# dbandstra/zang

Hardware: AMD Instinct MI355X
Metric: voice-samples/sec (higher is better)
Workload: dtype f32

## Files before the change

### zang_amd/csrc/dsp.hip.h

```cpp
#pragma once
#include "zmath.hip.h"
#include "lanes.hip.h"

template <int W>
struct PulseKT {
    typename LaneT<W>::U ifreq, brpt;
    typename LaneT<W>::F gdf2 , col, cc121, cc212;
};
using PulseK = PulseKT<1>;

__device__ __forceinline__ void pulse_setup_freq(PulseK &k, float srf, float freq) {
    const float gain = 0.7f;
    k.ifreq = zf32_to_u32(srf * freq);
    k.gdf2 = (gain / zutof23(k.ifreq)) * 2.0f;
    k.cc121 = k.gdf2 * (k.col - 1.0f) + gain;
    k.cc212 = k.gdf2 * k.col - gain;
}
__device__ __forceinline__ void pulse_setup_color(PulseK &k, float color) {
    k.brpt = zftou32(zclamp01(color));
    k.col = zutof23(k.brpt);
}
__device__ __forceinline__ void pulse_setup(PulseKT<1> &k, float srf, float freq, float color) {
    pulse_setup_color(k, color);
    pulse_setup_freq(k, srf, freq);
}
__device__ __forceinline__ void pulse_setup(PulseKT<2> &k, float srf, zf2 freq, zf2 color) {
    PulseK a, b;
    pulse_setup(a, srf, freq.x, color.x);
    pulse_setup(b, srf, freq.y, color.y);
    k.ifreq = zu2{a.ifreq, b.ifreq}; k.brpt = zu2{a.brpt, b.brpt};
    k.gdf2 = zf2{a.gdf2, b.gdf2}; k.col = zf2{a.col, b.col};
    k.cc121 = zf2{a.cc121, b.cc121}; k.cc212 = zf2{a.cc212, b.cc212};
}

__device__ __forceinline__ zf2 zutof23(zu2 x) { return zbits_f((x >> 9) | 0x3f800000u) - 1.0f; }

template <int W>
__device__ __forceinline__ typename LaneT<W>::F pulse_sample(const PulseKT<W> &k, typename LaneT<W>::U cnt,
                                                             typename LaneT<W>::F gain, typename LaneT<W>::F ngain) {
    using F = typename LaneT<W>::F;
    using M = typename LaneT<W>::M;
    const F p = zutof23(cnt);
    const M b0 = cnt < k.brpt;
    const M b1 = (cnt - k.ifreq) < k.brpt;
    const M b2 = cnt < k.ifreq;
    const F sg = zsel(b0, gain, ngain);
    const F ramp = k.gdf2 * zsel(b0, p, k.col - p) - sg;
    const F flat = zsel(b2, zsel(b0, k.cc121, k.cc212), sg);
    return zsel(b0 == b1, flat, ramp);
}

template <int W>
__device__ __forceinline__ typename LaneT<W>::F pulse_sample(const PulseKT<W> &k, typename LaneT<W>::U cnt) {
    using F = typename LaneT<W>::F;
    return pulse_sample<W>(k, cnt, zsplat<F>(0.7f), zsplat<F>(-0.7f));
}

#if !defined(__HIPCC_RTC__)
typedef unsigned long long PulseRoll;
__device__ __forceinline__ PulseRoll pulse_roll_init(const PulseK &k, uint32_t cnt) {
    return __builtin_amdgcn_ballot_w64((cnt - k.ifreq) < k.brpt);
}
__device__ __forceinline__ float pulse_sample_roll(const PulseK &k, uint32_t cnt, PulseRoll &prev, float gain = 0.7f, float ngain = -0.7f) {
#if defined(ZH_NO_PULSE_ROLL)
    (void)prev;
    return pulse_sample<1>(k, cnt, gain, ngain);
#endif
    const float p = zutof23(cnt);
    const bool b0 = cnt < k.brpt;
    const bool b2 = cnt < k.ifreq;
    const float sg = b0 ? gain : ngain;
    const float ramp = k.gdf2 * (b0 ? p : k.col - p) - sg;
    const float flat = b2 ? (b0 ? k.cc121 : k.cc212) : sg;
    const PulseRoll m0 = __builtin_amdgcn_ballot_w64(b0);
    const bool same = __builtin_amdgcn_inverse_ballot_w64(~(m0 ^ prev));
    prev = m0;
    return same ? flat : ramp;
}
#endif

template <class F> struct SvfOutT { F l, b, h; };
using SvfOut = SvfOutT<float>;
constexpr float kSvfDcOffset = 3.814697265625e-6f;
template <class F>
__device__ __forceinline__ SvfOutT<F> svf_core(F &l, F &b, F in, F cut, F res) {
    l += cut * b - kSvfDcOffset;
    b += cut * (in - b * res - l);
    l += cut * b;
    const F h = in - b * res - l;
    b += cut * h;
    return SvfOutT<F>{l, b, h};
}
template <class F> struct SvfMidT { F l, b1; };
using SvfMid = SvfMidT<float>;
template <class F>
__device__ __forceinline__ SvfMidT<F> svf_core_mid(F &l, F &b, F in, F cut, F res) {
    l += cut * b - kSvfDcOffset;
    b += cut * (in - b * res - l);
    l += cut * b;
    const F b1 = b;
    const F h = in - b * res - l;
    b += cut * h;
    return SvfMidT<F>{l, b1};
}
template <class F>
__device__ __forceinline__ SvfOutT<F> svf_finish(F l, F b1, F in, F cut, F res) {
    const F h = in - b1 * res - l;
    return SvfOutT<F>{l, b1 + cut * h, h};
}
template <class F>
__device__ __forceinline__ SvfOutT<F> svf_step(F &l, F &b, F input, F cut, F res) {
    return svf_core(l, b, input + kSvfDcOffset, cut, res);
}
template <class F>
__device__ __forceinline__ F svf_lowpass_into_zero(F l, F b) { return zsplat<F>(0.0f) + (l + b * 0.0f); }

__device__ __forceinline__ float pink_step(float (&b)[7], float white) {
    b[0] = 0.99886f * b[0] + white * 0.0555179f;
    b[1] = 0.99332f * b[1] + white * 0.0750759f;
    b[2] = 0.96900f * b[2] + white * 0.1538520f;
    b[3] = 0.86650f * b[3] + white * 0.3104856f;
    b[4] = 0.55000f * b[4] + white * 0.5329522f;
    b[5] = -0.7616f * b[5] - white * 0.0168980f;
    const float out = b[0] + b[1] + b[2] + b[3] + b[4] + b[5] + b[6] + white * 0.5362f;
    b[6] = white * 0.115926f;
    return out;
}
```

### zang_amd/csrc/nice.hip.h

```cpp
#pragma once
#include "common.hip.h"
#include "zmath.hip.h"
#include "dsp.hip.h"
#include "seq.hip.h"
#include "envelope.hip.h"
#include "voices.hip.h"

template <int W>
struct NiceLaneT {
    using F = typename LaneT<W>::F;
    using U = typename LaneT<W>::U;
    using M = typename LaneT<W>::M;
    U cnt;
    PulseKT<W> k;
    M bad;
    F g, ng;
    F l, b, cut, res;
    EnvLaneT<W, ZH_CURVE_CUBED> env;

    __device__ __forceinline__ void begin(float sample_rate, float srf, float sr8, F freq, F color, M note_on, M new_note) {
        bad = zor(freq < zsplat<F>(0.0f), freq > zsplat<F>(sr8));
        pulse_setup(k, srf, freq, color);
        const F zf = zsplat<F>(0.0f);
        const typename LaneT<W>::U zu = zsplatu<typename LaneT<W>::U>(0u);
        k.ifreq = zsel(bad, zu, k.ifreq); k.brpt = zsel(bad, zu, k.brpt);
        k.gdf2 = zsel(bad, zf, k.gdf2); k.cc121 = zsel(bad, zf, k.cc121); k.cc212 = zsel(bad, zf, k.cc212);
        g = zsel(bad, zf, zsplat<F>(0.7f)); ng = zsel(bad, zf, zsplat<F>(-0.7f));
        const F f8 = freq * 8.0f;
#pragma unroll
        for (int c = 0; c < W; c++) zput(cut, c, zclampf(zcutoff_from_frequency(zget(f8, c), sample_rate), 0.0f, 1.0f));
        res = zsplat<F>(1.0f - zclampf(0.7f, 0.0f, 1.0f));
        env.sample_rate = sample_rate;
        env.sustain_volume = zsplat<F>(0.8f);
        env.attack = CurvePT<W>{ZH_CURVE_CUBED, zsplat<F>(0.01f)};
        env.decay = CurvePT<W>{ZH_CURVE_CUBED, zsplat<F>(0.1f)};
        env.release = CurvePT<W>{ZH_CURVE_CUBED, zsplat<F>(0.5f)};
        env.note_on = note_on;
        env.begin(new_note);
    }

    __device__ __forceinline__ F osc(U c) const {
        const F pv = pulse_sample<W>(k, c, g, ng);
        return pv * 0.5f;
    }
    template <bool INTO_ZERO = false>
    __device__ __forceinline__ F tail_filter(F t0) {
        const SvfOutT<F> s = svf_step(l, b, t0, cut, res);
        if constexpr (INTO_ZERO) return s.l + s.b * 0.0f;
        else return svf_lowpass_into_zero(s.l, s.b);
    }
    __device__ __forceinline__ F tail_env() { return env.frame_masked(); }
    template <bool INTO_ZERO = false>
    __device__ __forceinline__ F tail(F t0) {
        const F t1 = tail_filter<INTO_ZERO>(t0);
        const F e0 = tail_env();
        return e0 * t1;
    }
    template <bool INTO_ZERO = false>
    __device__ __forceinline__ F frame() {
        const F t0 = osc(cnt);
        cnt = cnt + k.ifreq;
        return tail<INTO_ZERO>(t0);
    }
    __device__ __forceinline__ F env_quiet() const { return zbits_f(zbits_u(zsplat<F>(0.0f) + env.sustain_volume) & env.m_painted); }
    template <bool INTO_ZERO = false>
    __device__ __forceinline__ F frame_quiet(F e0) {
        const F t0 = osc(cnt);
        cnt = cnt + k.ifreq;
        return e0 * tail_filter<INTO_ZERO>(t0);
    }
    template <bool INTO_ZERO = false>
    __device__ __forceinline__ F frame_roll(PulseRoll &roll) { return tail<INTO_ZERO>(osc_next(roll)); }
    template <bool INTO_ZERO = false>
    __device__ __forceinline__ F frame_quiet_roll(F e0, PulseRoll &roll) { return e0 * tail_filter<INTO_ZERO>(osc_next(roll)); }
    __device__ __forceinline__ void roll_begin(PulseRoll &roll) const {
        static_assert(W == 1, "lane masks: one voice per lane");
        roll = pulse_roll_init(k, cnt);
    }
    __device__ __forceinline__ F osc_next(PulseRoll &roll) {
        const F pv = pulse_sample_roll(k, cnt, roll, g, ng);
        cnt = cnt + k.ifreq;
        return pv * 0.5f;
    }
};
using NiceLane = NiceLaneT<1>;

struct NiceArgs {
    float *color;
    uint32_t *cnt;
    float *fl, *fb;
    uint32_t *estate;
    float *et, *elast, *estart;
    uint32_t V;
    float sample_rate, srf, sr8;
    F32P freq;
    BoolP note_on, nic;
};

template <int W>
__device__ __forceinline__ void nice_load_state(NiceLaneT<W> &n, const NiceArgs &a, uint32_t v) {
    n.cnt = zload_u<W>(a.cnt, v); n.l = zload_f<W>(a.fl, v); n.b = zload_f<W>(a.fb, v);
    n.env.state = zload_u<W>(a.estate, v); n.env.t = zload_f<W>(a.et, v);
    n.env.last_value = zload_f<W>(a.elast, v); n.env.start = zload_f<W>(a.estart, v);
}
template <int W>
__device__ __forceinline__ void nice_load(NiceLaneT<W> &n, const NiceArgs &a, uint32_t v) {
    nice_load_state(n, a, v);
    n.begin(a.sample_rate, a.srf, a.sr8, zget_f32p<W>(a.freq, v), zload_f<W>(a.color, v), zget_boolp<W>(a.note_on, v), zget_boolp<W>(a.nic, v));
}
template <int W>
__device__ __forceinline__ void nice_store(NiceLaneT<W> &n, const NiceArgs &a, uint32_t v) {
    zstore_u<W>(a.cnt, v, n.cnt); zstore_f<W>(a.fl, v, n.l); zstore_f<W>(a.fb, v, n.b);
    zstore_u<W>(a.estate, v, n.env.state); zstore_f<W>(a.et, v, n.env.t);
    zstore_f<W>(a.elast, v, n.env.last_value); zstore_f<W>(a.estart, v, n.env.start);
}
```

### zang_amd/csrc/nice_mix.hip.h

```cpp
#pragma once
#include "nice.hip.h"
#ifndef ZH_K
#define ZH_K(name) name
#endif
constexpr int MIXF = 32;
constexpr int MIXS = 68;

template <int C, class G2>
__device__ __forceinline__ void nice_mix_gains(G2 &g2, const F32P &gain_l, const F32P &gain_r, bool live, uint32_t v, uint32_t wave, uint32_t rh) {
    typedef float f2 __attribute__((ext_vector_type(2)));
    if constexpr (C == 2) {
        __shared__ f2 gains[512];
        gains[threadIdx.x] = live ? f2{gain_l.get(v), gain_r.get(v)} : f2{0.0f, 0.0f};
        __syncthreads();
        const f2 *mine = &gains[wave * 64 + rh * 32];
#pragma unroll
        for (int j = 0; j < 32; j++) g2[j] = mine[j];
    }
}

template <int C, bool ROLL, int NW, class G2>
__device__ __forceinline__ void nice_mix_frames(NiceLane &n, PulseRoll &roll, const G2 &g2, float (*tile)[MIXS], float *__restrict__ pw_paint,
                                                size_t channel_stride, uint32_t rows, uint32_t wrow, uint32_t start, uint32_t end, uint32_t lane,
                                                uint32_t rf, uint32_t rh, float (*wsum)[NW ? NW : 4][C][MIXF] = nullptr, uint32_t wave = 0, uint32_t first = 0xFFFFFFFFu) {
    constexpr bool WG = NW != 0;
    uint32_t parity = 0;
    for (uint32_t f0 = first == 0xFFFFFFFFu ? start : first; f0 < end; f0 += MIXF) {
        const bool whole = f0 + MIXF <= end;
        if (!__any(n.env.mode == ENV_MODE_TOWARD)) {
            const float e0 = n.env_quiet();
            if (whole) {
#pragma unroll 4
                for (int k = 0; k < MIXF; k++) {
                    const float x = 0.0f + (ROLL ? n.template frame_quiet_roll<true>(e0, roll) : n.template frame_quiet<true>(e0));
                    tile[k][lane] = x;
                }
            } else {
                for (int k = 0; k < MIXF; k++) {
                    float x = 0.0f;
                    if (__builtin_amdgcn_readfirstlane((int)(f0 + k < end))) x = 0.0f + (ROLL ? n.template frame_quiet_roll<true>(e0, roll) : n.template frame_quiet<true>(e0));
                    tile[k][lane] = x;
                }
            }
        } else if (whole && n.env.quiet(MIXF)) {
            if (__all(n.env.mode == ENV_MODE_TOWARD)) {
#pragma unroll 4
                for (int k = 0; k < MIXF; k++) {
                    const float e0 = n.env.frame_masked_all_toward_quiet();
                    const float x = 0.0f + (ROLL ? n.template frame_quiet_roll<true>(e0, roll) : n.template frame_quiet<true>(e0));
                    tile[k][lane] = x;
                }
            } else {
#pragma unroll 4
                for (int k = 0; k < MIXF; k++) {
                    const float e0 = n.env.frame_masked_quiet();
                    const float x = 0.0f + (ROLL ? n.template frame_quiet_roll<true>(e0, roll) : n.template frame_quiet<true>(e0));
                    tile[k][lane] = x;
                }
            }
        } else if (whole) {
#pragma unroll 4
            for (int k = 0; k < MIXF; k++) {
                const float x = 0.0f + (ROLL ? n.template frame_roll<true>(roll) : n.template frame<true>());
                tile[k][lane] = x;
            }
        } else {
            for (int k = 0; k < MIXF; k++) {
                float x = 0.0f;
                if (__builtin_amdgcn_readfirstlane((int)(f0 + k < end))) x = 0.0f + (ROLL ? n.template frame_roll<true>(roll) : n.template frame<true>());
                tile[k][lane] = x;
            }
        }
        __builtin_amdgcn_fence(__ATOMIC_RELEASE, "wavefront");
        __builtin_amdgcn_wave_barrier();
        __builtin_amdgcn_fence(__ATOMIC_ACQUIRE, "wavefront");
        {
            const float4 *row4 = reinterpret_cast<const float4 *>(&tile[rf][rh * 32]);
            float row[32];
#pragma unroll
            for (int q = 0; q < 8; q++) { const float4 x = row4[q]; row[4 * q] = x.x; row[4 * q + 1] = x.y; row[4 * q + 2] = x.z; row[4 * q + 3] = x.w; }
            float sl, sr = 0.0f;
            if constexpr (C == 1) {
                sl = row[0];
#pragma unroll
                for (int j = 1; j < 32; j++) sl += row[j];
            } else {
                sl = row[0] * g2[0].x; sr = row[0] * g2[0].y;
#pragma unroll
                for (int j = 1; j < 32; j++) { sl += row[j] * g2[j].x; sr += row[j] * g2[j].y; }
            }
            const float hl = __shfl_down(sl, 32);
            const float hr = C == 2 ? __shfl_down(sr, 32) : 0.0f;
            if constexpr (!WG) {
                if (rh == 0 && f0 + rf < end) {
                    const uint32_t fr = (f0 - start) + rf;
                    float *pw = pw_paint + ((size_t)(fr / kMixGroupFrames) * rows + wrow) * kMixGroupFrames + (fr % kMixGroupFrames);
                    pw[0] = sl + hl;
                    if constexpr (C == 2) pw[channel_stride] = sr + hr;
                }
            } else {
                if (rh == 0) {
                    wsum[parity][wave][0][rf] = sl + hl;
                    if constexpr (C == 2) wsum[parity][wave][1][rf] = sr + hr;
                }
                __syncthreads();
                constexpr uint32_t FW = MIXF / (NW ? NW : 4);
                static_assert(kMixGroupFrames % FW == 0, "a wave's frames stay inside one frame group");
                const uint32_t q = lane % FW, c = lane / FW, fw = wave * FW + q;
                if (c < (uint32_t)C && f0 + fw < end) {
                    float t = wsum[parity][0][c][fw] + wsum[parity][1][c][fw];
#pragma unroll
                    for (int w = 2; w < (NW ? NW : 4); w++) t += wsum[parity][w][c][fw];
                    const uint32_t fr = (f0 - start) + fw;
                    pw_paint[c * channel_stride + ((size_t)(fr / kMixGroupFrames) * rows + wrow) * kMixGroupFrames + (fr % kMixGroupFrames)] = t;
                }
                parity ^= 1u;
            }
        }
        __builtin_amdgcn_fence(__ATOMIC_RELEASE, "wavefront");
        __builtin_amdgcn_wave_barrier();
    }
}

__device__ __forceinline__ void nice_silence(NiceLane &n) {
    n.k.ifreq = 0u; n.k.brpt = 0u; n.k.gdf2 = 0.0f; n.k.cc121 = 0.0f; n.k.cc212 = 0.0f; n.g = n.ng = 0.0f;
    n.l = n.b = 0.0f;
    n.env.mode = ENV_MODE_NONE; n.env.m_painted = 0u;
}

template <int C, bool ROLL, int NW = 0>
__global__ void __launch_bounds__(NW == 8 ? 512 : 256) ZH_K(k_nice_mix)(NiceArgs a, uint32_t start, uint32_t end, float *__restrict__ partials,
                                                                  F32P gain_l, F32P gain_r) {
    constexpr bool WG = NW != 0;
    constexpr int NWV = NW ? NW : 4;
    __shared__ float tile_all[NWV][MIXF][MIXS];
    __shared__ float wsum[WG ? 2 : 1][NWV][C][MIXF];
    const uint32_t v = blockIdx.x * (NWV * 64) + threadIdx.x;
    const uint32_t lane = threadIdx.x & 63, wave = threadIdx.x >> 6;
    float (*tile)[MIXS] = tile_all[wave];
    const uint32_t nframes = end - start;
    const uint32_t wave_global = WG ? blockIdx.x : blockIdx.x * NWV + wave;
    const uint32_t rows = WG ? gridDim.x : gridDim.x * NWV;
    const size_t channel_stride = (size_t)((nframes + kMixGroupFrames - 1) / kMixGroupFrames) * rows * kMixGroupFrames;
    const bool live = v < a.V;
    NiceLane n;
    nice_load(n, a, live ? v : a.V - 1);
    if (!live) nice_silence(n);
    const uint32_t rf = lane & (MIXF - 1), rh = lane >> 5;
    PulseRoll roll;
    n.roll_begin(roll);
    typedef float f2 __attribute__((ext_vector_type(2)));
    f2 g2[C == 2 ? 32 : 1];
    nice_mix_gains<C>(g2, gain_l, gain_r, live, v, wave, rh);
    nice_mix_frames<C, ROLL, NW>(n, roll, g2, tile, partials, channel_stride, rows, wave_global, start, end, lane, rf, rh, wsum, wave);
    if (live) nice_store(n, a, v);
}

constexpr int kNiceMixMaxBatch = 16;
struct NiceBatchArgs {
    NiceArgs a;
    F32P freq[kNiceMixMaxBatch];
    BoolP note_on[kNiceMixMaxBatch], nic[kNiceMixMaxBatch];
    uint32_t nb;
};
template <int C, bool ROLL, int NW = 0>
__global__ void __launch_bounds__(NW == 8 ? 512 : 256) ZH_K(k_nice_mix_batch)(const NiceBatchArgs b, uint32_t start, uint32_t end, float *__restrict__ partials,
                                                                        F32P gain_l, F32P gain_r) {
    constexpr bool WG = NW != 0;
    constexpr int NWV = NW ? NW : 4;
    __shared__ float tile_all[NWV][MIXF][MIXS];
    __shared__ float wsum[WG ? 2 : 1][NWV][C][MIXF];
    const NiceArgs &a = b.a;
    const uint32_t v = blockIdx.x * (NWV * 64) + threadIdx.x;
    const uint32_t lane = threadIdx.x & 63, wave = threadIdx.x >> 6;
    float (*tile)[MIXS] = tile_all[wave];
    const uint32_t nframes = end - start;
    const uint32_t wave_global = WG ? blockIdx.x : blockIdx.x * NWV + wave;
    const uint32_t rows = WG ? gridDim.x : gridDim.x * NWV;
    const size_t channel_stride = (size_t)((nframes + kMixGroupFrames - 1) / kMixGroupFrames) * rows * kMixGroupFrames;
    const bool live = v < a.V;
    const uint32_t vc = live ? v : a.V - 1;
    NiceLane n;
    nice_load_state(n, a, vc);
    const float color = a.color[vc];
    const uint32_t rf = lane & (MIXF - 1), rh = lane >> 5;
    typedef float f2 __attribute__((ext_vector_type(2)));
    f2 g2[C == 2 ? 32 : 1];
    nice_mix_gains<C>(g2, gain_l, gain_r, live, v, wave, rh);
    for (uint32_t k = 0; k < b.nb; k++) {
        n.begin(a.sample_rate, a.srf, a.sr8, b.freq[k].get(vc), color, b.note_on[k].get(vc), b.nic[k].get(vc));
        if (!live) nice_silence(n);
        PulseRoll roll;
        n.roll_begin(roll);
        nice_mix_frames<C, ROLL, NW>(n, roll, g2, tile, partials + (size_t)k * C * channel_stride, channel_stride, rows, wave_global, start, end, lane, rf, rh, wsum, wave);
    }
    if (live) nice_store(n, a, v);
}

void zh_nice_mix_fma_launch(int channels, bool roll, int nw, uint32_t blocks, hipStream_t st, const NiceArgs &a, uint32_t start, uint32_t end,
                            float *part, F32P gl, F32P gr);
void zh_nice_mix_batch_fma_launch(bool roll, int nw, uint32_t blocks, hipStream_t st, const NiceBatchArgs &bt, uint32_t start, uint32_t end,
                                  float *part, F32P gl, F32P gr);
```

### zang_amd/csrc/zmath.hip.h

```cpp
#pragma once
#include <hip/hip_runtime.h>
#if !defined(__HIPCC_RTC__)
#include <stdint.h>
#endif
#include "rtc_types.hip.h"

#define ZD __device__ __forceinline__

ZD uint32_t zf2u(float f) { return __float_as_uint(f); }
ZD float zu2f(uint32_t u) { return __uint_as_float(u); }

ZD uint32_t zf32_to_u32(float v) {
#if defined(__HIP_DEVICE_COMPILE__)
    uint32_t r;
    asm("v_cvt_u32_f32 %0, %1" : "=v"(r) : "v"(v));
    return r;
#else
    if (!(v == v)) return 0u;
    if (v <= 0.0f) return 0u;
    if (v >= 4294967296.0f) return 0xFFFFFFFFu;
    return (uint32_t)v;
#endif
}
ZD int32_t zf32_to_i32(float v) {
#if defined(__HIP_DEVICE_COMPILE__)
    int32_t r;
    asm("v_cvt_i32_f32 %0, %1" : "=v"(r) : "v"(v));
    return r;
#else
    if (!(v == v)) return 0;
    if (v <= -2147483648.0f) return INT32_MIN;
    if (v >= 2147483648.0f) return INT32_MAX;
    return (int32_t)v;
#endif
}

ZD float zminf(float a, float b) { return (a <= b || b != b) ? a : b; }
ZD float zmaxf(float a, float b) { return (a >= b || b != b) ? a : b; }
ZD float zclampf(float v, float lo, float hi) { return zmaxf(lo, zminf(v, hi)); }

__device__ static const int32_t ZM_IPIO2[66] = {
  0xA2F983, 0x6E4E44, 0x1529FC, 0x2757D1, 0xF534DD, 0xC0DB62,
  0x95993C, 0x439041, 0xFE5163, 0xABDEBB, 0xC561B7, 0x246E3A,
  0x424DD2, 0xE00649, 0x2EEA09, 0xD1921C, 0xFE1DEB, 0x1CB129,
  0xA73EE8, 0x8235F5, 0x2EBB44, 0x84E99C, 0x7026B4, 0x5F7E41,
  0x3991D6, 0x398353, 0x39F49C, 0x845F8B, 0xBDF928, 0x3B1FF8,
  0x97FFDE, 0x05980F, 0xEF2F11, 0x8B5A0A, 0x6D1F6D, 0x367ECF,
  0x27CB09, 0xB74F46, 0x3F669E, 0x5FEA2D, 0x7527BA, 0xC7EBE5,
  0xF17B3D, 0x0739F7, 0x8A5292, 0xEA6BFB, 0x5FB11F, 0x8D5D08,
  0x560330, 0x46FC7B, 0x6BABF0, 0xCFBC20, 0x9AF436, 0x1DA9E3,
  0x91615E, 0xE61B08, 0x659985, 0x5F14A0, 0x68408D, 0xFFD880,
  0x4D7327, 0x310606, 0x1556CA, 0x73A8C9, 0x60E27B, 0xC08C6B,
};
__device__ static const double ZM_PIO2[8] = {
  0x1.921fb40000000p+0,  0x1.4442d00000000p-24, 0x1.8469880000000p-48,
  0x1.8cc5160000000p-72, 0x1.01b8380000000p-96, 0x1.a252040000000p-120,
  0x1.3822280000000p-145, 0x1.9f31d00000000p-169,
};

struct ZRemLarge { int n; double y; };
__device__ __noinline__ __attribute__((pure)) static ZRemLarge zrem_pio2_large1(double x0, int e0) {
    int32_t jz, jv, carry, n, iq[20], i, j, k, q0, ih;
    const int32_t jk = 3;
    double z, fw, f[20], fq[20], q[20];
    jv = (e0 - 3) / 24; if (jv < 0) jv = 0;
    q0 = e0 - 24 * (jv + 1);
    for (i = 0; i <= jk; i++) f[i] = (double)ZM_IPIO2[jv + i];
    for (i = 0; i <= jk; i++) q[i] = x0 * f[i];
    jz = jk;
    for (;;) {
        for (i = 0, j = jz, z = q[jz]; j > 0; i++, j--) {
            fw = (double)(int32_t)(0x1p-24 * z);
            iq[i] = (int32_t)(z - 0x1p24 * fw);
            z = q[j - 1] + fw;
        }
        z = ldexp(z, q0);
        z -= 8.0 * floor(z * 0.125);
        n = (int32_t)z;
        z -= (double)n;
        ih = 0;
        if (q0 > 0) {
            i = iq[jz - 1] >> (24 - q0); n += i;
            iq[jz - 1] -= i << (24 - q0);
            ih = iq[jz - 1] >> (23 - q0);
        } else if (q0 == 0) ih = iq[jz - 1] >> 23;
        else if (z >= 0.5) ih = 2;
        if (ih > 0) {
            n += 1; carry = 0;
            for (i = 0; i < jz; i++) {
                j = iq[i];
                if (carry == 0) {
                    if (j != 0) { carry = 1; iq[i] = 0x1000000 - j; }
                } else iq[i] = 0xffffff - j;
            }
            if (q0 == 1) iq[jz - 1] &= 0x7fffff;
            else if (q0 == 2) iq[jz - 1] &= 0x3fffff;
            if (ih == 2) {
                z = 1.0 - z;
                if (carry != 0) z -= ldexp(1.0, q0);
            }
        }
        if (z == 0.0) {
            j = 0;
            for (i = jz - 1; i >= jk; i--) j |= iq[i];
            if (j == 0) {
                for (k = 1; iq[jk - k] == 0; k++) {}
                for (i = jz + 1; i <= jz + k; i++) {
                    f[i] = (double)ZM_IPIO2[jv + i];
                    q[i] = x0 * f[i];
                }
                jz += k;
                continue;
            }
        }
        break;
    }
    if (z == 0.0) {
        jz -= 1; q0 -= 24;
        while (iq[jz] == 0) { jz--; q0 -= 24; }
    } else {
        z = ldexp(z, -q0);
        if (z >= 0x1p24) {
            fw = (double)(int32_t)(0x1p-24 * z);
            iq[jz] = (int32_t)(z - 0x1p24 * fw);
            jz += 1; q0 += 24;
            iq[jz] = (int32_t)fw;
        } else iq[jz] = (int32_t)z;
    }
    fw = ldexp(1.0, q0);
    for (i = jz; i >= 0; i--) { q[i] = fw * (double)iq[i]; fw *= 0x1p-24; }
    for (i = jz; i >= 0; i--) {
        for (fw = 0.0, k = 0; k <= jk && k <= jz - i; k++) fw += ZM_PIO2[k] * q[i + k];
        fq[jz - i] = fw;
    }
    fw = 0.0;
    for (i = jz; i >= 0; i--) fw += fq[i];
    return ZRemLarge{n & 7, ih == 0 ? fw : -fw};
}

ZD int zrem_pio2f(float x, double *y) {
    const double toint = 1.5 / 2.220446049250313e-16, pio4 = 0x1.921fb6p-1,
                 invpio2 = 6.36619772367581382433e-01, pio2_1 = 1.57079631090164184570e+00,
                 pio2_1t = 1.58932547735281966916e-08;
    uint32_t ui = zf2u(x), ix = ui & 0x7fffffff;
    if (ix < 0x4dc90fdb) {
        double fn = (double)x * invpio2 + toint - toint;
        int n = (int32_t)fn;
        *y = x - fn * pio2_1 - fn * pio2_1t;
        if (*y < -pio4) { n--; fn--; *y = x - fn * pio2_1 - fn * pio2_1t; }
        else if (*y > pio4) { n++; fn++; *y = x - fn * pio2_1 - fn * pio2_1t; }
        return n;
    }
    if (ix >= 0x7f800000) { *y = x - x; return 0; }
    int sign = ui >> 31;
    int e0 = (int)(ix >> 23) - (0x7f + 23);
    const ZRemLarge big = zrem_pio2_large1((double)zu2f(ix - ((uint32_t)e0 << 23)), e0);
    if (sign) { *y = -big.y; return -big.n; }
    *y = big.y;
    return big.n;
}

template <bool MAYBE_LARGE = true>
ZD int zreduce_pio2f(float x, uint32_t ix, double &y) {
    const double invpio2 = 6.36619772367581382433e-01,
                 pio2_1 = 1.57079631090164184570e+00, pio2_1t = 1.58932547735281966916e-08,
                 toint = 1.5 / 2.220446049250313e-16;
    const double xd = (double)x;
    const double fnm = __builtin_fma(xd, invpio2, toint);
    const double fn = fnm - toint;
    int n = (int)(uint32_t)__double_as_longlong(fnm);
    y = __builtin_fma(-fn, pio2_1t, __builtin_fma(-fn, pio2_1, xd));
    if (MAYBE_LARGE && __builtin_expect(__builtin_amdgcn_ballot_w64(ix > 0x4dc90fdau) != 0, 0)) {
        if (ix > 0x4dc90fdau) n = zrem_pio2f(x, &y);
    }
    return n;
}

ZD void zsincos_kernels(double y, float &sv, float &cv) {
    const double S1 = -0x15555554cbac77.0p-55, S2 = 0x111110896efbb2.0p-59, S3 = -0x1a00f9e2cae774.0p-65, S4 = 0x16cd878c3b46a7.0p-71;
    const double C0 = -0x1ffffffd0c5e81.0p-54, C1 = 0x155553e1053a42.0p-57, C2 = -0x16c087e80f1e27.0p-62, C3 = 0x199342e0ee5069.0p-68;
    const double z = y * y, w = z * z, s = z * y;
    sv = (float)__builtin_fma(s * w, __builtin_fma(z, S4, S3), __builtin_fma(s, __builtin_fma(z, S2, S1), y));
    cv = (float)__builtin_fma(w * z, __builtin_fma(z, C3, C2), __builtin_fma(w, C1, __builtin_fma(z, C0, 1.0)));
}

constexpr uint32_t kZSinOneLeafOdd = 0x40406406u;
constexpr float kZSinNoLargeBelow = 4.0e8f;
template <bool MAYBE_LARGE = true>
ZD float zsinf(float x) {
    const uint32_t ux = zf2u(x), ix = ux & 0x7fffffff;
    double y;
    const int n = zreduce_pio2f<MAYBE_LARGE>(x, ix, y);
    float sv, cv;
    zsincos_kernels(y, sv, cv);
    float r = zu2f(zf2u((n & 1) ? cv : sv) ^ ((uint32_t)(n & 2) << 30));
    r = zu2f(zf2u(r) - (uint32_t)(ix == kZSinOneLeafOdd));
    if (ix < 0x39800000) r = x;
    return r;
}

ZD float zsinf_tol(float x) {
    const float inv_pi = 0.31830988618379067154f, pi_hi = 3.14159274101257324219f, pi_lo = -8.74227765734758577e-8f;
    if (__builtin_expect(__builtin_amdgcn_ballot_w64(!(__builtin_fabsf(x) < 1048576.0f)) != 0, 0)) {
        if (!(__builtin_fabsf(x) < 1048576.0f)) return zsinf<true>(x);
    }
    const float kf = __builtin_rintf(x * inv_pi);
    float r = __builtin_fmaf(-kf, pi_hi, x);
    r = __builtin_fmaf(-kf, pi_lo, r);
    const float z = r * r;
    float p = -2.50521083854417187751e-8f;
    p = __builtin_fmaf(p, z, 2.75573192239858906526e-6f);
    p = __builtin_fmaf(p, z, -1.98412698412698412698e-4f);
    p = __builtin_fmaf(p, z, 8.33333333333333333333e-3f);
    p = __builtin_fmaf(p, z, -1.66666666666666666667e-1f);
    const float sv = __builtin_fmaf(r * z, p, r);
    return zu2f(zf2u(sv) ^ ((uint32_t)(int)kf << 31));
}

template <bool MAYBE_LARGE = true>
ZD float zcosf(float x) {
    const uint32_t ux = zf2u(x), ix = ux & 0x7fffffff;
    double y;
    const int n = zreduce_pio2f<MAYBE_LARGE>(x, ix, y);
    float sv, cv;
    zsincos_kernels(y, sv, cv);
    float r = zu2f(zf2u((n & 1) ? sv : cv) ^ ((uint32_t)((n + 1) & 2) << 30));
    return r;
}

ZD float zatanf(float x) {
    const float aT0 = 3.3333328366e-01f, aT1 = -1.9999158382e-01f, aT2 = 1.4253635705e-01f,
                aT3 = -1.0648017377e-01f, aT4 = 6.1687607318e-02f;
    const uint32_t ux = zf2u(x), ix = ux & 0x7fffffff;
    const bool sign = (ux >> 31) != 0;
    const float ax = fabsf(x);
    const bool r0 = ix < 0x3f300000, r1 = ix < 0x3f980000, r2 = ix < 0x401c0000;
    const float c = r0 ? 0.5f : (r1 ? 1.0f : 1.5f);
    const float num = r2 ? ax - c : -1.0f;
    const float den = r2 ? 1.0f + c * ax : ax;
    const float hi = r1 ? (r0 ? 4.6364760399e-01f : 7.8539812565e-01f) : (r2 ? 9.8279368877e-01f : 1.5707962513e+00f);
    const float lo = r1 ? (r0 ? 5.0121582440e-09f : 3.7748947079e-08f) : (r2 ? 3.4473217170e-08f : 7.5497894159e-08f);
    const bool direct = ix < 0x3ee00000;
    const float rc = __builtin_amdgcn_rcpf(den);
    const float q = num * rc;
    const float xr = direct ? x : __builtin_fmaf(__builtin_fmaf(-den, q, num), rc, q);
    const float z = xr * xr;
    const float w = z * z;
    const float s1 = z * (aT0 + w * (aT2 + w * aT4));
    const float s2 = w * (aT1 + w * aT3);
    const float t = xr * (s1 + s2);
    const float zz = hi - ((t - lo) - xr);
    float r = direct ? xr - t : (sign ? -zz : zz);
    if (ix < 0x39800000) r = x;
    if (ix >= 0x4c800000) {
        const float big = 1.5707962513e+00f + 0x1p-120f;
        r = (x != x) ? x : (sign ? -big : big);
    }
    return r;
}

ZD float zlogf(float x) {
    const float ln2_hi = 6.9313812256e-01f, ln2_lo = 9.0580006145e-06f, Lg1 = 0xaaaaaa.0p-24f,
                Lg2 = 0xccce13.0p-25f, Lg3 = 0x91e9ee.0p-25f, Lg4 = 0xf89e26.0p-26f;
    uint32_t ix = zf2u(x);
    int k = 0;
    if (ix < 0x00800000 || ix >> 31) {
        if (ix << 1 == 0) return -__builtin_inff();
        if (ix >> 31) return __builtin_nanf("");
        k -= 25; x *= 0x1p25f; ix = zf2u(x);
    } else if (ix >= 0x7f800000) return x;
    else if (ix == 0x3f800000) return 0;
    ix += 0x3f800000 - 0x3f3504f3;
    k += (int)(ix >> 23) - 0x7f;
    ix = (ix & 0x007fffff) + 0x3f3504f3;
    x = zu2f(ix);
    float f = x - 1.0f;
    float s = f / (2.0f + f);
    float z = s * s;
    float w = z * z;
    float t1 = w * (Lg2 + w * Lg4);
    float t2 = z * (Lg1 + w * Lg3);
    float R = t2 + t1;
    float hfsq = 0.5f * f * f;
    float dk = (float)k;
    return s * (hfsq + R) + dk * ln2_lo - hfsq + f + dk * ln2_hi;
}

ZD float zexpf(float x) {
    const float ln2hi = 6.9314575195e-1f, ln2lo = 1.4286067653e-6f, invln2 = 1.4426950216e+0f,
                P1 = 1.6666625440e-1f, P2 = -2.7667332906e-3f;
    uint32_t hx = zf2u(x);
    int sign = hx >> 31, k;
    float hi, lo;
    hx &= 0x7fffffff;
    if (x != x) return x;
    if (hx >= 0x42aeac50) {
        if (hx > 0x7f800000) return x;
        if (hx >= 0x42b17218 && !sign) return x * 0x1p127f;
        if (sign && hx >= 0x42cff1b5) return 0;
    }
    if (hx > 0x3eb17218) {
        if (hx > 0x3f851592) k = (int)(invln2 * x + (sign ? -0.5f : 0.5f));
        else k = 1 - sign - sign;
        float fk = (float)k;
        hi = x - fk * ln2hi;
        lo = fk * ln2lo;
        x = hi - lo;
    } else if (hx > 0x39000000) {
        k = 0; hi = x; lo = 0;
    } else return 1 + x;
    float xx = x * x;
    float c = x - xx * (P1 + xx * P2);
    float y = 1 + (x * c / (2 - c) - lo + hi);
    if (k == 0) return y;
    return ldexpf(y, k);
}

ZD float zpowf_pos(float x, float y) {
    if (y == 0 || x == 1) return 1;
    if (y != y) return __builtin_nanf("");
    if (y == 1) return x;
    if (__builtin_isinf(y)) {
        if ((x < 1) == (y > 0)) return 0;
        return __builtin_inff();
    }
    if (y == 0.5f) return sqrtf(x);
    if (y == -0.5f) return 1 / sqrtf(x);
    float ay = fabsf(y);
    float yi = truncf(ay);
    float yf = ay - yi;
    if (yi >= 2147483648.0f) return zexpf(y * zlogf(x));
    float a1 = 1.0f;
    int ae = 0;
    if (yf != 0) {
        if (yf > 0.5f) { yf -= 1; yi += 1; }
        a1 = zexpf(yf * zlogf(x));
    }
    int xe;
    float x1 = frexpf(x, &xe);
    for (int32_t i = (int32_t)yi; i != 0; i >>= 1) {
        if (xe < -(1 << 9) || (1 << 9) < xe) { ae += xe; break; }
        if (i & 1) { a1 *= x1; ae += xe; }
        x1 *= x1;
        xe <<= 1;
        if (x1 < 0.5f) { x1 += x1; xe -= 1; }
    }
    if (y < 0) { a1 = 1 / a1; ae = -ae; }
    return ldexpf(a1, ae);
}

ZD float zpowf(float x, float y) {
    if (y == 0 || x == 1) return 1;
    if (x != x || y != y) return __builtin_nanf("");
    if (y == 1) return x;
    if (x == 0) {
        bool y_odd_int = false;
        if (fabsf(y) < 16777216.0f) { const float yi = truncf(y); y_odd_int = (yi == y) && ((int32_t)yi & 1); }
        if (y < 0) return y_odd_int ? copysignf(__builtin_inff(), x) : __builtin_inff();
        return y_odd_int ? x : 0.0f;
    }
    if (__builtin_isinf(y)) {
        if (x == -1) return 1;
        if ((fabsf(x) < 1) == (y > 0)) return 0;
        return __builtin_inff();
    }
    if (__builtin_isinf(x)) {
        if (x < 0) {
            const float ny = -y;
            bool odd = false;
            if (fabsf(ny) < 16777216.0f) { const float yi = truncf(ny); odd = (yi == ny) && ((int32_t)yi & 1); }
            if (ny < 0) return odd ? -__builtin_inff() : __builtin_inff();
            return odd ? -0.0f : 0.0f;
        }
        return y < 0 ? 0.0f : __builtin_inff();
    }
    if (y == 0.5f) return sqrtf(x);
    if (y == -0.5f) return 1 / sqrtf(x);
    float ay = fabsf(y);
    float yi = truncf(ay);
    float yf = ay - yi;
    if (yf != 0 && x < 0) return __builtin_nanf("");
    if (yi >= 2147483648.0f) return zexpf(y * zlogf(x));
    float a1 = 1.0f;
    int ae = 0;
    if (yf != 0) {
        if (yf > 0.5f) { yf -= 1; yi += 1; }
        a1 = zexpf(yf * zlogf(x));
    }
    int xe;
    float x1 = frexpf(x, &xe);
    for (int32_t i = (int32_t)yi; i != 0; i >>= 1) {
        if (xe < -(1 << 9) || (1 << 9) < xe) { ae += xe; break; }
        if (i & 1) { a1 *= x1; ae += xe; }
        x1 *= x1;
        xe <<= 1;
        if (x1 < 0.5f) { x1 += x1; xe -= 1; }
    }
    if (y < 0) { a1 = 1 / a1; ae = -ae; }
    return ldexpf(a1, ae);
}

struct ZXoshiro { uint64_t s0, s1, s2, s3; };

ZD uint64_t zrotl64(uint64_t x, int k) { return (x << k) | (x >> (64 - k)); }

ZD void zxoshiro_seed(ZXoshiro &r, uint64_t seed) {
    uint64_t sm = seed, o[4];
#pragma unroll
    for (int i = 0; i < 4; i++) {
        sm += 0x9e3779b97f4a7c15ull;
        uint64_t z = sm;
        z = (z ^ (z >> 30)) * 0xbf58476d1ce4e5b9ull;
        z = (z ^ (z >> 27)) * 0x94d049bb133111ebull;
        o[i] = z ^ (z >> 31);
    }
    r.s0 = o[0]; r.s1 = o[1]; r.s2 = o[2]; r.s3 = o[3];
}
ZD uint64_t zxoshiro_next(ZXoshiro &r) {
    uint64_t result = zrotl64(r.s0 + r.s3, 23) + r.s0;
    uint64_t t = r.s1 << 17;
    r.s2 ^= r.s0; r.s3 ^= r.s1; r.s1 ^= r.s2; r.s0 ^= r.s3;
    r.s2 ^= t;
    r.s3 = zrotl64(r.s3, 45);
    return result;
}
ZD float zrandom_float32(ZXoshiro &r) {
    const uint64_t rnd = zxoshiro_next(r);
    const uint32_t hi = (uint32_t)(rnd >> 32);
    uint32_t lz;
    asm("v_ffbh_u32 %0, %1" : "=v"(lz) : "v"(hi));
    if (__builtin_expect(__builtin_amdgcn_ballot_w64(hi == 0u) != 0, 0)) {
        if (hi == 0u) {
            lz = rnd ? (uint32_t)__clzll((long long)rnd) : 64u;
            if (lz >= 41) {
                uint64_t r2 = zxoshiro_next(r);
                lz = 41 + (r2 ? (uint32_t)__clzll((long long)r2) : 64u);
                if (lz == 41 + 64) lz += (uint32_t)__clz((int)((uint32_t)zxoshiro_next(r) | 0x7FFu));
            }
        }
    }
    return zu2f(((126u - lz) << 23) | ((uint32_t)rnd & 0x7FFFFFu));
}

ZD float zclamp01(float v) { return v < 0.0f ? 0.0f : (v > 1.0f ? 1.0f : v); }
ZD float zutof23(uint32_t x) { return zu2f((x >> 9) | 0x3f800000u) - 1.0f; }
ZD uint32_t zftou32(float v) { return zf32_to_u32(v * 4294967296.0f * 0.99995f); }

ZD float zcutoff_from_frequency(float frequency, float sample_rate) {
    const float v = 2.0f * (1.0f - zcosf(3.14159265358979323846f * frequency / sample_rate));
    return sqrtf(zclampf(v, 0.0f, 1.0f));
}
```

Before: 1657 billion.

## Fold pulse gain into constants, speculate finite filter state, use alignbit for zutof23

Folds the 0.5 oscillator output scale into the pulse constants and gains at setup, which removes a multiply per sample. Each mix chunk now runs speculatively with the filter's `b*0` term dropped, assuming the band state stays finite. If any lane ends with a non-finite `b`, the chunk is replayed from a saved copy of the lane state using the exact path. zutof23 now builds its mantissa bits with a single v_alignbit instead of a shift and an or. The costs are a per-chunk state copy, a wave-wide finiteness check, and larger code from instantiating both variants.

```diff
diff --git a/zang_amd/csrc/dsp.hip.h b/zang_amd/csrc/dsp.hip.h
--- a/zang_amd/csrc/dsp.hip.h
+++ b/zang_amd/csrc/dsp.hip.h
@@ -33,7 +33,7 @@
     k.cc121 = zf2{a.cc121, b.cc121}; k.cc212 = zf2{a.cc212, b.cc212};
 }
 
-__device__ __forceinline__ zf2 zutof23(zu2 x) { return zbits_f((x >> 9) | 0x3f800000u) - 1.0f; }
+__device__ __forceinline__ zf2 zutof23(zu2 x) { return zbits_f(zu2{zutof23_bits(x.x), zutof23_bits(x.y)}) - 1.0f; }
 
 template <int W>
 __device__ __forceinline__ typename LaneT<W>::F pulse_sample(const PulseKT<W> &k, typename LaneT<W>::U cnt,
diff --git a/zang_amd/csrc/nice.hip.h b/zang_amd/csrc/nice.hip.h
--- a/zang_amd/csrc/nice.hip.h
+++ b/zang_amd/csrc/nice.hip.h
@@ -26,6 +26,7 @@
         k.ifreq = zsel(bad, zu, k.ifreq); k.brpt = zsel(bad, zu, k.brpt);
         k.gdf2 = zsel(bad, zf, k.gdf2); k.cc121 = zsel(bad, zf, k.cc121); k.cc212 = zsel(bad, zf, k.cc212);
         g = zsel(bad, zf, zsplat<F>(0.7f)); ng = zsel(bad, zf, zsplat<F>(-0.7f));
+        k.gdf2 = k.gdf2 * 0.5f; k.cc121 = k.cc121 * 0.5f; k.cc212 = k.cc212 * 0.5f; g = g * 0.5f; ng = ng * 0.5f;
         const F f8 = freq * 8.0f;
 #pragma unroll
         for (int c = 0; c < W; c++) zput(cut, c, zclampf(zcutoff_from_frequency(zget(f8, c), sample_rate), 0.0f, 1.0f));
@@ -40,39 +41,40 @@
     }
 
     __device__ __forceinline__ F osc(U c) const {
-        const F pv = pulse_sample<W>(k, c, g, ng);
-        return pv * 0.5f;
+        return pulse_sample<W>(k, c, g, ng);
     }
-    template <bool INTO_ZERO = false>
+    template <bool INTO_ZERO = false, bool B_FINITE = false>
     __device__ __forceinline__ F tail_filter(F t0) {
         const SvfOutT<F> s = svf_step(l, b, t0, cut, res);
-        if constexpr (INTO_ZERO) return s.l + s.b * 0.0f;
+        static_assert(INTO_ZERO || !B_FINITE, "B_FINITE drops the mix of a paint into a zero");
+        if constexpr (INTO_ZERO && B_FINITE) return s.l;
+        else if constexpr (INTO_ZERO) return s.l + s.b * 0.0f;
         else return svf_lowpass_into_zero(s.l, s.b);
     }
     __device__ __forceinline__ F tail_env() { return env.frame_masked(); }
-    template <bool INTO_ZERO = false>
+    template <bool INTO_ZERO = false, bool B_FINITE = false>
     __device__ __forceinline__ F tail(F t0) {
-        const F t1 = tail_filter<INTO_ZERO>(t0);
+        const F t1 = tail_filter<INTO_ZERO, B_FINITE>(t0);
         const F e0 = tail_env();
         return e0 * t1;
     }
-    template <bool INTO_ZERO = false>
+    template <bool INTO_ZERO = false, bool B_FINITE = false>
     __device__ __forceinline__ F frame() {
         const F t0 = osc(cnt);
         cnt = cnt + k.ifreq;
-        return tail<INTO_ZERO>(t0);
+        return tail<INTO_ZERO, B_FINITE>(t0);
     }
     __device__ __forceinline__ F env_quiet() const { return zbits_f(zbits_u(zsplat<F>(0.0f) + env.sustain_volume) & env.m_painted); }
-    template <bool INTO_ZERO = false>
+    template <bool INTO_ZERO = false, bool B_FINITE = false>
     __device__ __forceinline__ F frame_quiet(F e0) {
         const F t0 = osc(cnt);
         cnt = cnt + k.ifreq;
-        return e0 * tail_filter<INTO_ZERO>(t0);
+        return e0 * tail_filter<INTO_ZERO, B_FINITE>(t0);
     }
-    template <bool INTO_ZERO = false>
-    __device__ __forceinline__ F frame_roll(PulseRoll &roll) { return tail<INTO_ZERO>(osc_next(roll)); }
-    template <bool INTO_ZERO = false>
-    __device__ __forceinline__ F frame_quiet_roll(F e0, PulseRoll &roll) { return e0 * tail_filter<INTO_ZERO>(osc_next(roll)); }
+    template <bool INTO_ZERO = false, bool B_FINITE = false>
+    __device__ __forceinline__ F frame_roll(PulseRoll &roll) { return tail<INTO_ZERO, B_FINITE>(osc_next(roll)); }
+    template <bool INTO_ZERO = false, bool B_FINITE = false>
+    __device__ __forceinline__ F frame_quiet_roll(F e0, PulseRoll &roll) { return e0 * tail_filter<INTO_ZERO, B_FINITE>(osc_next(roll)); }
     __device__ __forceinline__ void roll_begin(PulseRoll &roll) const {
         static_assert(W == 1, "lane masks: one voice per lane");
         roll = pulse_roll_init(k, cnt);
@@ -80,7 +82,7 @@
     __device__ __forceinline__ F osc_next(PulseRoll &roll) {
         const F pv = pulse_sample_roll(k, cnt, roll, g, ng);
         cnt = cnt + k.ifreq;
-        return pv * 0.5f;
+        return pv;
     }
 };
 using NiceLane = NiceLaneT<1>;
diff --git a/zang_amd/csrc/nice_mix.hip.h b/zang_amd/csrc/nice_mix.hip.h
--- a/zang_amd/csrc/nice_mix.hip.h
+++ b/zang_amd/csrc/nice_mix.hip.h
@@ -19,6 +19,55 @@
     }
 }
 
+template <bool ROLL, bool SPEC>
+__device__ __forceinline__ void nice_mix_chunk(NiceLane &n, PulseRoll &roll, float (*tile)[MIXS], uint32_t f0, uint32_t end, uint32_t lane) {
+    const bool whole = f0 + MIXF <= end;
+    if (!__any(n.env.mode == ENV_MODE_TOWARD)) {
+        const float e0 = n.env_quiet();
+        if (whole) {
+#pragma unroll 4
+            for (int k = 0; k < MIXF; k++) {
+                const float x = 0.0f + (ROLL ? n.template frame_quiet_roll<true, SPEC>(e0, roll) : n.template frame_quiet<true, SPEC>(e0));
+                tile[k][lane] = x;
+            }
+        } else {
+            for (int k = 0; k < MIXF; k++) {
+                float x = 0.0f;
+                if (__builtin_amdgcn_readfirstlane((int)(f0 + k < end))) x = 0.0f + (ROLL ? n.template frame_quiet_roll<true, SPEC>(e0, roll) : n.template frame_quiet<true, SPEC>(e0));
+                tile[k][lane] = x;
+            }
+        }
+    } else if (whole && n.env.quiet(MIXF)) {
+        if (__all(n.env.mode == ENV_MODE_TOWARD)) {
+#pragma unroll 4
+            for (int k = 0; k < MIXF; k++) {
+                const float e0 = n.env.frame_masked_all_toward_quiet();
+                const float x = 0.0f + (ROLL ? n.template frame_quiet_roll<true, SPEC>(e0, roll) : n.template frame_quiet<true, SPEC>(e0));
+                tile[k][lane] = x;
+            }
+        } else {
+#pragma unroll 4
+            for (int k = 0; k < MIXF; k++) {
+                const float e0 = n.env.frame_masked_quiet();
+                const float x = 0.0f + (ROLL ? n.template frame_quiet_roll<true, SPEC>(e0, roll) : n.template frame_quiet<true, SPEC>(e0));
+                tile[k][lane] = x;
+            }
+        }
+    } else if (whole) {
+#pragma unroll 4
+        for (int k = 0; k < MIXF; k++) {
+            const float x = 0.0f + (ROLL ? n.template frame_roll<true, SPEC>(roll) : n.template frame<true, SPEC>());
+            tile[k][lane] = x;
+        }
+    } else {
+        for (int k = 0; k < MIXF; k++) {
+            float x = 0.0f;
+            if (__builtin_amdgcn_readfirstlane((int)(f0 + k < end))) x = 0.0f + (ROLL ? n.template frame_roll<true, SPEC>(roll) : n.template frame<true, SPEC>());
+            tile[k][lane] = x;
+        }
+    }
+}
+
 template <int C, bool ROLL, int NW, class G2>
 __device__ __forceinline__ void nice_mix_frames(NiceLane &n, PulseRoll &roll, const G2 &g2, float (*tile)[MIXS], float *__restrict__ pw_paint,
                                                 size_t channel_stride, uint32_t rows, uint32_t wrow, uint32_t start, uint32_t end, uint32_t lane,
@@ -26,50 +75,12 @@
     constexpr bool WG = NW != 0;
     uint32_t parity = 0;
     for (uint32_t f0 = first == 0xFFFFFFFFu ? start : first; f0 < end; f0 += MIXF) {
-        const bool whole = f0 + MIXF <= end;
-        if (!__any(n.env.mode == ENV_MODE_TOWARD)) {
-            const float e0 = n.env_quiet();
-            if (whole) {
-#pragma unroll 4
-                for (int k = 0; k < MIXF; k++) {
-                    const float x = 0.0f + (ROLL ? n.template frame_quiet_roll<true>(e0, roll) : n.template frame_quiet<true>(e0));
-                    tile[k][lane] = x;
-                }
-            } else {
-                for (int k = 0; k < MIXF; k++) {
-                    float x = 0.0f;
-                    if (__builtin_amdgcn_readfirstlane((int)(f0 + k < end))) x = 0.0f + (ROLL ? n.template frame_quiet_roll<true>(e0, roll) : n.template frame_quiet<true>(e0));
-                    tile[k][lane] = x;
-                }
-            }
-        } else if (whole && n.env.quiet(MIXF)) {
-            if (__all(n.env.mode == ENV_MODE_TOWARD)) {
-#pragma unroll 4
-                for (int k = 0; k < MIXF; k++) {
-                    const float e0 = n.env.frame_masked_all_toward_quiet();
-                    const float x = 0.0f + (ROLL ? n.template frame_quiet_roll<true>(e0, roll) : n.template frame_quiet<true>(e0));
-                    tile[k][lane] = x;
-                }
-            } else {
-#pragma unroll 4
-                for (int k = 0; k < MIXF; k++) {
-                    const float e0 = n.env.frame_masked_quiet();
-                    const float x = 0.0f + (ROLL ? n.template frame_quiet_roll<true>(e0, roll) : n.template frame_quiet<true>(e0));
-                    tile[k][lane] = x;
-                }
-            }
-        } else if (whole) {
-#pragma unroll 4
-            for (int k = 0; k < MIXF; k++) {
-                const float x = 0.0f + (ROLL ? n.template frame_roll<true>(roll) : n.template frame<true>());
-                tile[k][lane] = x;
-            }
-        } else {
-            for (int k = 0; k < MIXF; k++) {
-                float x = 0.0f;
-                if (__builtin_amdgcn_readfirstlane((int)(f0 + k < end))) x = 0.0f + (ROLL ? n.template frame_roll<true>(roll) : n.template frame<true>());
-                tile[k][lane] = x;
-            }
+        const NiceLane n0 = n;
+        const PulseRoll roll0 = roll;
+        nice_mix_chunk<ROLL, true>(n, roll, tile, f0, end, lane);
+        if (__builtin_expect(__any(!__builtin_isfinite(n.b)), 0)) {
+            n = n0; roll = roll0;
+            nice_mix_chunk<ROLL, false>(n, roll, tile, f0, end, lane);
         }
         __builtin_amdgcn_fence(__ATOMIC_RELEASE, "wavefront");
         __builtin_amdgcn_wave_barrier();
diff --git a/zang_amd/csrc/zmath.hip.h b/zang_amd/csrc/zmath.hip.h
--- a/zang_amd/csrc/zmath.hip.h
+++ b/zang_amd/csrc/zmath.hip.h
@@ -443,7 +443,8 @@
 }
 
 ZD float zclamp01(float v) { return v < 0.0f ? 0.0f : (v > 1.0f ? 1.0f : v); }
-ZD float zutof23(uint32_t x) { return zu2f((x >> 9) | 0x3f800000u) - 1.0f; }
+ZD uint32_t zutof23_bits(uint32_t x) { return __builtin_amdgcn_alignbit(0x7fu, x, 9u); }
+ZD float zutof23(uint32_t x) { return zu2f(zutof23_bits(x)) - 1.0f; }
 ZD uint32_t zftou32(float v) { return zf32_to_u32(v * 4294967296.0f * 0.99995f); }
 
 ZD float zcutoff_from_frequency(float frequency, float sample_rate) {
```

Result: no change. 1645 billion (median of 2 runs) (-0.7%).
